# milos-agathon/forge3d

Hardware: AMD Instinct MI355X
Metric: Msamples/s (W*H*spp/s) at 1920x1080, 11616 spp (8 spp/frame x 1452 frames timed); SSIM vs golden (higher is better)
Workload: dtype f32

## Files before the change

forge3d_amd/_native.py:

```python
from __future__ import annotations

import ctypes as C
import os
from pathlib import Path

import numpy as np

_PKG = Path(__file__).resolve().parent
LIB_PATH = _PKG / "libf3dhip.so"

STATUS_OK, STATUS_VALUE, STATUS_RENDER, STATUS_UPLOAD, STATUS_DEVICE = 0, 1, 2, 3, 4
ABI_VERSION = 6
FRAMES_IN_FLIGHT_AUTO = 0xFFFFFFFF

_EARTH = {"flat": 0, "sphere": 1, "ellipsoid": 2, "wgs84": 2}
_REFRACTION = {"none": 0, "bennett": 1, "saemundsson": 2, "effective_radius": 3}


class Desc(C.Structure):
    _fields_ = [
        ("struct_size", C.c_uint32),
        ("heights", C.c_void_p), ("dem_width", C.c_uint32), ("dem_height", C.c_uint32),
        ("spacing_x", C.c_float), ("spacing_z", C.c_float), ("exaggeration", C.c_float),
        ("albedo", C.c_float * 3),
# ... 196 lines not shown
    ("f3d_scene_cache_entries", C.c_uint32, []),
    ("f3d_wavefront_render", C.c_int, [C.c_void_p, C.c_uint32, C.c_uint32, C.c_uint32, C.c_uint32, C.c_uint32, C.c_int32,
                                       C.c_void_p, C.c_char_p, C.c_size_t]),
    ("f3d_aether_bake", C.c_int, [C.c_void_p, C.c_void_p, C.c_void_p, C.c_void_p, C.c_void_p, C.c_void_p, _P(C.c_double),
                                  C.c_char_p, C.c_size_t]),
    ("f3d_smoke_render", C.c_int, [C.c_void_p, C.c_void_p, C.c_void_p, C.c_void_p, _P(C.c_double), C.c_char_p, C.c_size_t]),
    ("f3d_smoke_step", C.c_int, [C.c_void_p, C.c_void_p, C.c_void_p, C.c_uint32, C.c_uint32, _P(C.c_double), C.c_char_p, C.c_size_t]),
    ("f3d_aether_reference_render", C.c_int, [C.c_void_p, C.c_void_p, C.c_char_p, C.c_size_t]),
    ("f3d_smoke_composite", C.c_int, [C.c_void_p, C.c_void_p, _P(C.c_double), C.c_char_p, C.c_size_t]),
    ("f3d_session_fingerprint", C.c_int, [C.c_void_p, C.c_void_p, C.c_uint32]),
    ("f3d_session_mesh_tree", C.c_int, [C.c_void_p, _P(C.c_uint32), C.c_void_p, C.c_size_t, C.c_void_p, C.c_size_t, C.c_char_p, C.c_size_t]),
    ("f3d_session_rearm", C.c_int, [C.c_void_p, _P(RearmDesc), C.c_char_p, C.c_size_t]),
    ("f3d_session_render", C.c_int, [C.c_void_p, _P(Out), C.c_char_p, C.c_size_t]),
    ("f3d_session_reaim", C.c_int, [C.c_void_p, _P(ReaimDesc), C.c_char_p, C.c_size_t]),
    ("f3d_session_remesh", C.c_int, [C.c_void_p, _P(RemeshDesc), C.c_char_p, C.c_size_t]),
    ("f3d_session_reterrain", C.c_int, [C.c_void_p, _P(ReterrainDesc), C.c_char_p, C.c_size_t]),
    ("f3d_session_query", C.c_int, [C.c_void_p, _P(QueryDesc), C.c_char_p, C.c_size_t]),
    ("f3d_session_raster", C.c_int, [C.c_void_p, _P(RasterDesc), C.c_char_p, C.c_size_t]),
    ("f3d_session_horizon", C.c_int, [C.c_void_p, _P(HorizonDesc), C.c_char_p, C.c_size_t]),
    ("f3d_session_irradiation", C.c_int, [C.c_void_p, _P(IrradiationDesc), C.c_char_p, C.c_size_t]),
    ("f3d_session_drape", C.c_int, [C.c_void_p, _P(DrapeDesc), C.c_char_p, C.c_size_t]),
    ("f3d_session_draped", C.c_int, [C.c_void_p, _P(C.c_uint32)]),
    ("f3d_session_certificates", C.c_int, [C.c_void_p, _P(C.c_uint64)]),
    ("f3d_session_debug_wave_times", C.c_int, [C.c_void_p, C.c_void_p]),
    ("f3d_session_halo", C.c_int, [C.c_void_p, C.c_int32, C.c_int32, _P(C.c_void_p), _P(C.c_uint64)]),
    ("f3d_session_resolve", C.c_int, [C.c_void_p, C.c_uint32, C.c_void_p, C.c_void_p, C.c_void_p, C.c_void_p,
                                      _P(C.c_int32), C.c_char_p, C.c_size_t]),
    ("f3d_session_resolve_device", C.c_int, [C.c_void_p, C.c_uint32, C.c_void_p, C.c_void_p, C.c_void_p,
                                             C.c_void_p, C.c_char_p, C.c_size_t]),
    ("f3d_session_setup_ms", C.c_int, [C.c_void_p, _P(C.c_double), C.c_uint32]),
    ("f3d_session_info", C.c_int, [C.c_void_p, _P(C.c_uint64), _P(C.c_uint64), _P(C.c_uint64), _P(C.c_uint32),
                                   _P(C.c_uint32)]),
    ("f3d_session_kernel_timing", C.c_int, [C.c_void_p, C.c_int32, _P(C.c_double), _P(C.c_uint32)]),
    ("f3d_session_sample_lanes", C.c_uint32, [C.c_void_p]),
    ("f3d_session_row_costs", C.c_int, [C.c_void_p, _P(C.c_float), C.c_uint32, C.c_char_p, C.c_size_t]),
    ("f3d_session_primary_start", C.c_void_p, [C.c_void_p]),
    ("f3d_smoke_set_stream", None, [C.c_void_p]),
    ("f3d_smoke_wait_fields_read", C.c_int, [C.c_void_p]),
    ("f3d_smoke_seq_create", C.c_int, [C.c_void_p, C.c_void_p, _P(C.c_void_p), C.c_char_p, C.c_size_t]),
    ("f3d_smoke_seq_destroy", None, [C.c_void_p]),
    ("f3d_smoke_seq_streams", C.c_int, [C.c_void_p, _P(C.c_void_p), _P(C.c_void_p)]),
    ("f3d_smoke_seq_step", C.c_int, [C.c_void_p, C.c_void_p, C.c_void_p, C.c_void_p, C.c_uint32, C.c_uint32, _P(C.c_double), C.c_char_p, C.c_size_t]),
    ("f3d_smoke_seq_render", C.c_int, [C.c_void_p, C.c_void_p, C.c_void_p, C.c_void_p, C.c_void_p, _P(C.c_double), C.c_char_p, C.c_size_t]),
    ("f3d_smoke_seq_composite", C.c_int, [C.c_void_p, C.c_void_p, C.c_void_p, _P(C.c_double), C.c_char_p, C.c_size_t]),
    ("f3d_smoke_seq_stats", C.c_int, [C.c_void_p, C.c_void_p, C.c_char_p, C.c_size_t]),
    ("f3d_halo_rows", C.c_uint32, []),
# ... 325 lines not shown
```

forge3d_amd/csrc/f3d_frame.h:

```cpp
#pragma once
#include "f3d_launch.h"
#include "f3d_shade.h"
#include "f3d_query.h"
#include "f3d_raster.h"
#include "f3d_horizon.h"
#include "f3d_irradiation.h"
#include "f3d_lds.h"
#include "f3d_tiles.h"

namespace f3d {

template <uint32_t S = 1u>
__device__ __forceinline__ bool tile_pixel(const FrameParams &P, uint32_t &gx, uint32_t &gy, uint32_t &tile,
                                           const uint32_t *order = nullptr, uint32_t wg = 0xFFFFFFFFu) {
    if (wg == 0xFFFFFFFFu) wg = blockIdx.x;
    constexpr TileDims shape = tile_shape<S>();
    const uint32_t rows = P.band_end - P.band_begin;
    const TileGrid grid = tile_grid(P.cam.width, rows, shape);
    if (!workgroup_tile(wg, grid, P.tile_map, order, tile)) return false;
    tile_lane_pixel(tile, threadIdx.x, grid.tiles_x, P.band_begin, shape, gx, gy);
    return gx < P.cam.width && gy < P.band_end;
}
__device__ __forceinline__ bool tile_pixel(const FrameParams &P, uint32_t &gx, uint32_t &gy) {
    uint32_t tile;
    return tile_pixel<1u>(P, gx, gy, tile);
}
template <uint32_t S>
__device__ __forceinline__ void lane_pixel(const FrameParams &P, uint32_t tile, uint32_t &gx, uint32_t &gy) {
    constexpr TileDims shape = tile_shape<S>();
    tile_lane_pixel(tile, lane_now(), tiles_across(P.cam.width, shape), P.band_begin, shape, gx, gy);
}
// ... 458 lines not shown
    if (__ballot(redo) != 0ull) {
        LdsPending pend = make_pending(lds, P.terrain);
        if (redo) {
            m2 = fix_pixel(P, gx, gy, rec, pixels, pend);
            atomicAdd(&P.fix_count[2], 1u);
        }
    }
    if (P.collect_stats != 0u) publish_window_stats(P, active, m2);
}

__global__ __launch_bounds__(kWave) void k_trace_init(const FrameParams P) {
    uint32_t gx, gy;
    if (!tile_pixel(P, gx, gy)) return;
    const size_t lp = (size_t)(gy - P.row_begin) * P.cam.width + gx;
    P.head[lp] = first_head(P, P.gbuffer_n[lp]);
}

__device__ __forceinline__ bool head_neighbourhood_empty(const FrameParams &P, uint32_t gx, uint32_t gy) {
    const uint32_t lane = lane_now();
    const uint32_t x0 = gx - (lane & 7u), y0 = gy - (lane >> 3);
    const uint32_t x_last = (x0 + 7u < P.cam.width ? x0 + 7u : P.cam.width - 1u), y_last = (y0 + 7u < P.band_end ? y0 + 7u : P.band_end - 1u);
    const uint32_t xa = x0 >= kSpatialReachLo ? x0 - kSpatialReachLo : 0u, ya = y0 >= kSpatialReachLo ? y0 - kSpatialReachLo : 0u;
    static_assert(8u + kSpatialReachLo + kSpatialReachHi <= 16u, "the 16 x 16 raster below covers the tile's reach");
    const uint32_t xb = x_last + kSpatialReachHi < P.cam.width ? x_last + kSpatialReachHi : P.cam.width - 1u;
    const uint32_t yb = y_last + kSpatialReachHi < P.cam.height ? y_last + kSpatialReachHi : P.cam.height - 1u;
    const uint32_t *words = reinterpret_cast<const uint32_t *>(P.res_in);
    uint32_t some = 0u;
#pragma unroll
    for (uint32_t i = 0u; i < 4u; i++) {
        const uint32_t k = lane + 64u * i, bx = xa + (k & 15u), by = ya + (k >> 4);
        if (bx <= xb && by <= yb) some |= words[4u * reservoir_index(P, bx, by) + 1u] & ~kLightTypeBit;
    }
    return __ballot(some != 0u) == 0ull;
}

__global__ __launch_bounds__(kWave) void k_head(const FrameParams P) {
    uint32_t gx, gy, tile;
    const bool active = tile_pixel<1u>(P, gx, gy, tile);
    if (tile == 0xFFFFFFFFu) return;
#if !defined(F3D_NO_EMPTY_HEAD)
    if (P.frame_index > 0u && head_neighbourhood_empty(P, gx, gy)) {
        if (active) {
            const size_t ri = reservoir_index(P, gx, gy), lp = (size_t)(gy - P.row_begin) * P.cam.width + gx;
            const PackedReservoir self = P.res_in[ri];
            P.res_out[ri] = PackedReservoir{0.0f, self.m_lt, 0.0f, self.target_pdf};
            FrameHead h;
            h.centre_hit = P.gbuffer_n[lp].w != 0.0f;
            h.prev_valid = false;
            h.reuse_w = 1.0f;
            h.rng = 0u;
            P.head[lp] = pack_head(h);
        }
        return;
    }
#endif
    if (active) P.head[(size_t)(gy - P.row_begin) * P.cam.width + gx] = pack_head(frame_head<true>(P, gx, gy));
}

template <uint32_t S, bool MESH, bool DRAPE>
__device__ __forceinline__ void frame_wave(const FrameParams &P, uint32_t *lds) {
    const unsigned long long t_start = wall_clock64();
    typename PendingFor<MESH>::type pend{make_pending(lds, P.terrain)};
    uint32_t gx = 0u, gy = 0u, tile;
    const bool active = tile_pixel<S>(P, gx, gy, tile, P.tile_order);
    float m2 = 0.0f;
    if constexpr (S == 1u) {
        if (active) m2 = frame_pixel<DRAPE>(P, gx, gy, pend);
        if (P.collect_stats != 0u) publish_window_stats(P, active, m2);
    } else {
        m2 = frame_lanes<S, DRAPE>(P, tile, active, pend);
        if (P.collect_stats != 0u) publish_window_stats(P, active && (lane_now() & (S - 1u)) == 0u, m2);
    }
    if (lane_now() == 0u) {
        const unsigned long long t_end = wall_clock64();
        if (P.tile_cost && tile != 0xFFFFFFFFu) P.tile_cost[tile] = (uint32_t)(t_end - t_start);
#if defined(F3D_WAVE_TIMES)
        if (P.wave_times) {
            P.wave_times[2u * blockIdx.x] = t_start;
            P.wave_times[2u * blockIdx.x + 1u] = t_end;
        }
#endif
    }
}
template <int VARIANT, int MIN_WAVES = 1, uint32_t S = 1u, bool MESH = false>
__global__ __launch_bounds__(kWave, MIN_WAVES) void k_frame(const FrameParams P) {
    __shared__ __attribute__((aligned(16))) uint32_t lds[kLdsWords];
    frame_wave<S, MESH, false>(P, lds);
}
template <int MIN_WAVES, uint32_t S, bool MESH>
__global__ __launch_bounds__(kWave, MIN_WAVES) void k_frame_drape(const FrameParams P) {
    __shared__ __attribute__((aligned(16))) uint32_t lds[kLdsWords];
    frame_wave<S, MESH, true>(P, lds);
}

__global__ __launch_bounds__(kWave) void k_gbuffer(const FrameParams P, float4 *gbuffer_n, float *depth) {
    __shared__ __attribute__((aligned(16))) uint32_t lds[kLdsWords];
    LdsPending pend = make_pending(lds, P.terrain);
    uint32_t gx, gy;
    if (tile_pixel(P, gx, gy)) gbuffer_pixel(P, gx, gy, gbuffer_n, depth, pend);
}

__global__ __launch_bounds__(kWave) void k_rearm(const RearmParams R) {
    const FrameParams &P = R.frame;
    uint32_t gx, gy;
    if (!tile_pixel(P, gx, gy)) return;
    rearm_certificate(P, gx, gy, P.gbuffer_n, R.depth);
    rearm_clear(R, gx, gy);
    rearm_head(P, gx, gy, P.gbuffer_n[(size_t)(gy - P.row_begin) * P.cam.width + gx]);
}

__global__ __launch_bounds__(kWave) void k_reaim(const RearmParams R) {
    __shared__ __attribute__((aligned(16))) uint32_t lds[kLdsWords];
    LdsPending pend = make_pending(lds, R.frame.terrain);
    uint32_t gx, gy;
    if (tile_pixel(R.frame, gx, gy)) reaim_pixel(R, gx, gy, pend);
// ... 184 lines not shown
```

forge3d_amd/csrc/f3d_host.hip:

```cpp
#include <hip/hip_runtime.h>

#include <atomic>
#include <deque>
#include <exception>
#include <memory>
#include <map>
#include <mutex>
#include <new>
#include <unordered_map>

#include <unistd.h>

#include "f3d_bvh_refit.h"
#include "f3d_devmem.h"
#include "f3d_launch.h"
#include "f3d_lbvh.h"
#include "f3d_meshgrid.h"
#include "f3d_retable.h"
#include "f3d_setup.h"
#include "f3d_tables.h"
#include "f3d_tiles.h"

using namespace f3d;

namespace {

void hip_check(hipError_t e, const char *what) {
    if (e != hipSuccess) fail(F3D_STATUS_DEVICE, "HIP failure in %s: %s", what, hipGetErrorString(e));
}

struct DeviceGuard {
    int prev = -1;
    bool switched = false;
    explicit DeviceGuard(int device) {
        if (device < 0 || hipGetDevice(&prev) != hipSuccess) return;
        if (prev != device) switched = hipSetDevice(device) == hipSuccess;
    }
    ~DeviceGuard() {
        if (switched) (void)hipSetDevice(prev);
    }
};

template <class Body>
int c_abi(char *err, size_t errlen, Body &&body) {
// ... 92 lines not shown
    bool owns_reservoirs = false;
    uint8_t *d_rgba = nullptr;
    float *d_albedo = nullptr, *d_normal = nullptr;
    int variant = 0;
    AetherDev aether{};
    bool require_valid_reservoirs = false;
    f3d_terrain_ref_desc desc{};
    bool rendered = false;
    double reaim_seconds = 0.0;
    uint64_t budget = 0;
    struct Band {
        uint32_t begin = 0, end = 0;
        hipStream_t stream = nullptr;
        bool edge = true;
        hipEvent_t done[2] = {nullptr, nullptr};
        int64_t last = -1;
        bool unjoined = false;
    };
    std::vector<Band> bands;
    std::vector<hipStream_t> band_streams;
    hipEvent_t fork = nullptr;
    uint32_t *tile_cost = nullptr, *tile_order = nullptr;
    int64_t cost_frame = -1, order_frame = -1;
    uint32_t fd_frames = 0;
    bool wavefront = false;
    uint32_t wf_quorum = 0;
    int64_t trace_first = -1;
    uint32_t trace_count = 0;
    bool timing = false;
    std::vector<std::pair<hipEvent_t, hipEvent_t>> events;
    ~f3d_session() {
        for (auto &e : events) {
            (void)hipEventDestroy(e.first);
            (void)hipEventDestroy(e.second);
        }
        for (auto &b : bands)
            for (hipEvent_t e : b.done)
                if (e) (void)hipEventDestroy(e);
        if (fork) (void)hipEventDestroy(fork);
        for (hipStream_t st : band_streams) (void)hipStreamDestroy(st);
        if (host_stats) (void)hipHostFree(host_stats);
        for (auto &link : peer)
            for (void *base : link.opened)
                if (base) (void)hipIpcCloseMemHandle(base);
        if (halo_flags) (void)hipFree(halo_flags);
        mem.release();
    }
};

namespace {

void plan_bands(f3d_session &s, uint32_t want, uint32_t want_streams);

void aether_sun_terms(AetherDev &A, const f3d_terrain_ref_desc &d) {
    A.sun_intensity = aether_clamp_scale(f_clamp(d.sun_intensity, 0.0f, 65504.0f));
    A.exposure = aether_clamp_scale(f_clamp(d.exposure, 0.0f, 65504.0f));
}

uint32_t same_sun_of(const FrameParams &P) {
    return f_bits(P.light.wi.x) == f_bits(P.light.wi_reuse.x) && f_bits(P.light.wi.y) == f_bits(P.light.wi_reuse.y) &&
                   f_bits(P.light.wi.z) == f_bits(P.light.wi_reuse.z) ? 1u : 0u;
}

void upload_aether(f3d_session &s, const f3d_aether_luts &L, const f3d_terrain_ref_desc &d) {
    auto bad = [](const char *why) { fail(F3D_STATUS_RENDER, "invalid AETHER PT settings: %s", why); };
    const float scalars[9] = {L.turbidity, L.ozone_du, L.mie_g, L.bottom_radius_m, L.top_radius_m, L.rayleigh_scale_height_m,
                              L.mie_scale_height_m, L.max_aerial_distance_m, L.ground_albedo};
    for (float v : scalars)
        if (!std::isfinite(v)) bad("all scalar parameters must be finite");
    if (!(L.turbidity >= 1.0f && L.turbidity <= 10.0f)) bad("turbidity must be in [1, 10]");
    if (!(L.ozone_du >= 0.0f && L.ozone_du <= 600.0f)) bad("ozone must be in [0, 600] DU");
    if (!(L.mie_g >= 0.0f && L.mie_g <= 0.99f)) bad("mie_g must be in [0, 0.99]");
    if (L.bottom_radius_m <= 0.0f || L.top_radius_m <= L.bottom_radius_m) bad("top radius must exceed a positive bottom radius");
    if (L.rayleigh_scale_height_m <= 0.0f || L.mie_scale_height_m <= 0.0f || L.max_aerial_distance_m <= 0.0f)
        bad("scale heights and aerial distance must be positive");
    if (!(L.ground_albedo >= 0.0f && L.ground_albedo <= 1.0f)) bad("ground albedo must be in [0, 1]");
    if (L.scattering_orders < 2u || L.scattering_orders > 8u) bad("scattering_orders must be in [2, 8]");
    const uint32_t dims[9] = {L.transmittance_mu, L.transmittance_height, L.scattering_mu_view, L.scattering_mu_sun,
                              L.scattering_height, L.scattering_nu, L.aerial_distance, L.aerial_mu_view, L.aerial_height};
// ... 313 lines not shown

    if (s.mem.device_bytes > s.budget)
        fail(F3D_STATUS_RENDER,
             "terrain PT exceeds the memory budget before rendering: tracked total %llu (host-visible %llu) > limit %llu",
             (unsigned long long)s.mem.device_bytes, (unsigned long long)s.mem.host_visible_peak,
             (unsigned long long)s.budget);

    plan_bands(s, opts ? opts->bands : 0u, opts ? opts->band_streams : 0u);
    const bool lpt = s.bands.size() == 1 && ((s.variant / 1000) % 10 == 0);
    if ((s.variant / 1000) % 10 == 4) P.tile_map = 2u;
    if (lpt) {
        uint32_t grid = 0;
        const uint32_t tiles = frame_tile_count(P, &grid);
        s.tile_cost = (uint32_t *)s.mem.alloc((size_t)tiles * sizeof(uint32_t), "tile costs");
        s.tile_order = (uint32_t *)s.mem.alloc((size_t)(grid ? grid : 1u) * sizeof(uint32_t), "tile order");
        hip_check(hipMemsetAsync(s.tile_cost, 0, (size_t)tiles * sizeof(uint32_t), s.stream), "tile cost clear");
    }

    P.frame_index = 0;
    P.res_in = s.res[1];
    P.res_out = s.res[0];
    P.collect_stats = 0;
    hip_check(launch_gbuffer(P, s.gbuffer_n, s.depth, s.stream), "g-buffer pass");
    if (s.fd_frames) {
        P.band_begin = s.row_begin;
        P.band_end = s.row_end;
        hip_check(launch_trace_init(P, s.stream), "trace prediction init");
    }
    clock.lap(kSetupPasses);
}

template <class Launch>
void ordered_timed_launch(f3d_session &s, hipStream_t stream, uint32_t frame, Launch &&launch) {
    constexpr int64_t kOrderEvery = 4;
    FrameParams &P = s.params;
    P.tile_cost = s.tile_cost;
    P.tile_order = nullptr;
    if (s.tile_cost && s.cost_frame >= 0) {
        if (s.order_frame < 0 || s.cost_frame - s.order_frame >= kOrderEvery) {
            hip_check(launch_tile_order(P, s.tile_cost, s.tile_order, stream), "tile order kernel");
            s.order_frame = s.cost_frame;
        }
        P.tile_order = s.tile_order;
    }
    hipEvent_t e0 = nullptr, e1 = nullptr;
    if (s.timing) {
// ... 15 lines not shown
    FrameParams &P = s.params;
    P.frame_index = frame;
    P.res_out = s.res[frame & 1u];
    P.res_in = s.res[(frame & 1u) ^ 1u];
    P.collect_stats = collect ? 1u : 0u;
    P.band_begin = b.begin;
    P.band_end = b.end;
    const bool piped = b.stream != s.stream;
    if (b.last != (int64_t)frame - 1 && !(b.last < 0 && frame == 0u) && piped)
        fail(F3D_STATUS_VALUE, "frames must be enqueued in order (band %zu is at frame %lld, frame %u wanted)", index,
             (long long)b.last, frame);
    if (piped) {
        hip_check(hipStreamWaitEvent(b.stream, s.fork, 0), "band fork");
        for (int d = -1; d <= 1; d += 2) {
            const size_t n = index + (size_t)d;
            if (n >= s.bands.size() || frame == 0u) continue;
            f3d_session::Band &nb = s.bands[n];
            if (nb.last != (int64_t)frame - 1 && nb.last != (int64_t)frame)
                fail(F3D_STATUS_VALUE, "frames must be enqueued in order (band %zu is at frame %lld, frame %u wanted)", n,
                     (long long)nb.last, frame);
            if (nb.stream != b.stream) hip_check(hipStreamWaitEvent(b.stream, nb.done[(frame - 1u) & 1u], 0), "band wait");
        }
    }
    if (P.sample_lanes > 1u) hip_check(launch_head(P, b.stream), "frame head kernel");
    ordered_timed_launch(s, b.stream, frame, [&] { hip_check(launch_frame(P, s.variant, b.stream), "frame kernel"); });
    if (piped) {
        hip_check(hipEventRecord(b.done[frame & 1u], b.stream), "band done");
        b.unjoined = true;
    }
    b.last = frame;
    P.band_begin = s.row_begin;
    P.band_end = s.row_end;
}

void fork_bands(f3d_session &s, bool clear_stats) {
    if (clear_stats) hip_check(hipMemsetAsync(s.stats, 0, 2 * sizeof(uint32_t), s.stream), "stats clear");
    if (s.fork) hip_check(hipEventRecord(s.fork, s.stream), "band fork");
}

void join_bands(f3d_session &s, bool edges_only = false) {
    for (auto &b : s.bands)
        if (b.unjoined && (b.edge || !edges_only)) {
            hip_check(hipStreamWaitEvent(s.stream, b.done[b.last & 1], 0), "band join");
            b.unjoined = false;
        }
}

void refuse_draped(const f3d_session &s, const char *path) {
// ... 517 lines not shown
        const double t_setup = now_s();
        hip_check(hipStreamSynchronize(s->stream), "setup sync");
        out->setup_seconds = now_s() - t_setup + s->reaim_seconds;
        s->reaim_seconds = 0.0;
        render_loop(*s, out);
    });
}

int f3d_session_certificates(f3d_session *s, uint64_t out[2]) {
    if (!s || !out) return F3D_STATUS_VALUE;
    try {
        DeviceGuard guard(s->device);
        join_bands(*s);
        hip_check(hipStreamSynchronize(s->stream), "certificates");
        const size_t px = (size_t)s->rows * s->width;
        auto dev = [&](const void *ptr, size_t bytes) -> uint64_t {
            if (!ptr || !bytes) return 0ull;
            std::vector<uint8_t> host(bytes);
            hip_check(hipMemcpy(host.data(), ptr, bytes, hipMemcpyDeviceToHost), "certificate download");
            return hash_bytes(host.data(), bytes, 0x243F6A8885A308D3ull);
        };
        out[0] = dev(s->params.sun_clear, px * sizeof(float2));
        out[1] = dev(s->params.primary_start, px * sizeof(uint2));
        return F3D_STATUS_OK;
    } catch (...) {
        return F3D_STATUS_DEVICE;
    }
}

int f3d_session_debug_wave_times(f3d_session *s, void *device_buffer) {
#if defined(F3D_WAVE_TIMES)
    if (!s) return F3D_STATUS_VALUE;
    s->params.wave_times = (unsigned long long *)device_buffer;
    return F3D_STATUS_OK;
#else
    (void)s;
    (void)device_buffer;
    return F3D_STATUS_VALUE;
#endif
}

int f3d_terrain_ref_render(const f3d_terrain_ref_desc *desc, f3d_terrain_ref_out *out, char *err, size_t errlen) {
    if (err && errlen) err[0] = 0;
    if (!desc || !out) return F3D_STATUS_VALUE;
    f3d_session *s = new (std::nothrow) f3d_session();
    if (!s) return F3D_STATUS_DEVICE;
// ... 205 lines not shown
```

forge3d_amd/csrc/f3d_host_update.h:

```cpp
#pragma once

namespace {

struct Update {
    f3d_session &s;
    const bool cam;
    const double t_host = now_s();
    f3d_terrain_ref_desc d;
    FrameParams U{};
    bool require_valid = false;

    Update(f3d_session &session, const f3d_session_rearm_desc &r, const f3d_session_reaim_desc *aim, const char *done)
        : s(session), cam(aim != nullptr) {
        if (aim) check_struct_size(*aim, "f3d_session_reaim_desc");
        check_struct_size(r, "f3d_session_rearm_desc");
        if (s.peer[0].connected || s.peer[1].connected)
            fail(F3D_STATUS_VALUE, "a session with peer halos cannot be %s: the frame counters its neighbours poll only rise", done);
        d = s.desc;
        d.sun_azimuth_deg = r.sun_azimuth_deg;
        d.sun_elevation_deg = r.sun_elevation_deg;
        d.sun_intensity = r.sun_intensity;
        for (int c = 0; c < 3; c++) d.sun_color[c] = r.sun_color[c];
        d.exposure = r.exposure;
        d.env_intensity = r.env_intensity;
// ... 35 lines not shown
        s.require_valid_reservoirs = require_valid;
        s.desc = d;
        s.desc.mesh_vertices = nullptr;
        s.desc.mesh_indices = nullptr;

        join_bands(s);
        P.band_begin = s.row_begin;
        P.band_end = s.row_end;
        P.frame_index = 0;
        P.trace_first = 0u;
        P.res_in = s.res[1];
        P.res_out = s.res[0];
        P.collect_stats = 0;
        P.tile_order = nullptr;
        P.tile_cost = nullptr;
        RearmParams R{};
        R.frame = P;
        R.gbuffer_n = s.gbuffer_n;
        R.depth = s.depth;
        R.res[0] = s.res[0];
        R.res[1] = s.res[1];
        R.tile_cost = s.tile_cost;
        R.tiles = s.tile_cost ? frame_tile_count(P, nullptr) : 0u;
        if (cam) hip_check(launch_reaim(R, s.stream), "re-aim kernel");
        else hip_check(launch_rearm(R, s.stream), "re-arm kernel");
        s.cost_frame = s.order_frame = -1;
        s.rendered = false;
        s.trace_first = -1;
        s.trace_count = 0;
        for (auto &b : s.bands) {
            b.last = -1;
            b.unjoined = false;
        }
        s.reaim_seconds = cam ? now_s() - t_host : 0.0;
    }
};

void check_budget(const f3d_session &s, uint64_t planned, const char *update, const char *brings) {
    if (planned > s.budget)
        fail(F3D_STATUS_RENDER, "%s exceeds the memory budget: %s the tracked total to %llu > limit %llu", update, brings,
             (unsigned long long)planned, (unsigned long long)s.budget);
}

void rearm(f3d_session &s, const f3d_session_rearm_desc &r) {
    Update u(s, r, nullptr, "re-armed");
    u.validate();
    u.apply();
}
// ... 225 lines not shown
```

forge3d_amd/csrc/f3d_kernels.hip:

```cpp
#include <type_traits>

#include "f3d_frame.h"

namespace f3d {

void horizon_table_dims(uint32_t cell_w, uint32_t cell_h, uint32_t *level, uint32_t *bx, uint32_t *bz) {
    *level = horizon_block_level(cell_w, cell_h);
    *bx = (cell_w + (1u << *level) - 1u) >> *level;
    *bz = (cell_h + (1u << *level) - 1u) >> *level;
}
hipError_t launch_horizon_build(const TerrainDev &terrain, float *table, hipStream_t stream) {
    HorizonBuildParams B{};
    B.terrain = terrain;
    B.terrain.horizon = nullptr;
    horizon_table_dims(terrain.cell_w, terrain.cell_h, &B.level, &B.bx, &B.bz);
    B.table = table;
    hipLaunchKernelGGL(k_horizon_build, dim3(((B.bx + 7u) >> 3) * ((B.bz + 7u) >> 3)), dim3(kWave), 0, stream, B);
    return hipGetLastError();
}
static inline TileGrid band_tiles(const FrameParams &p, uint32_t lanes) {
    return tile_grid(p.cam.width, p.band_end - p.band_begin, tile_shape(lanes));
}
static inline uint32_t frame_grid(const FrameParams &p, uint32_t lanes = 1u) { return launch_size(band_tiles(p, lanes), p.tile_map); }

// ... 104 lines not shown
    hipLaunchKernelGGL(k_trace_init, dim3(frame_grid(p)), dim3(kWave), 0, stream, p);
    return hipGetLastError();
}
hipError_t launch_merge(const FrameParams &p, hipStream_t stream) {
    if (frame_grid(p) == 0u) return hipSuccess;
    hipLaunchKernelGGL(k_merge, dim3(frame_grid(p)), dim3(kWave), 0, stream, p);
    return hipGetLastError();
}
hipError_t launch_tile_order(const FrameParams &p, const uint32_t *cost, uint32_t *order, hipStream_t stream) {
    const TileGrid tiles = band_tiles(p, sample_lanes_of(p));
    TileOrderParams B{cost, order, tiles.tiles_x, tiles.tiles_y};
    hipLaunchKernelGGL(k_tile_order, dim3(kNumXcd), dim3(1024), 0, stream, B);
    return hipGetLastError();
}
uint32_t frame_tile_count(const FrameParams &p, uint32_t *grid) {
    const uint32_t lanes = sample_lanes_of(p);
    if (grid) *grid = frame_grid(p, lanes);
    return band_tiles(p, lanes).count();
}
hipError_t launch_gbuffer(const FrameParams &p, float4 *gbuffer_n, float *depth, hipStream_t stream) {
    hipLaunchKernelGGL(k_gbuffer, dim3(frame_grid(p)), dim3(kWave), 0, stream, p, gbuffer_n, depth);
    return hipGetLastError();
}
hipError_t launch_rearm(const RearmParams &p, hipStream_t stream) {
    if (frame_grid(p.frame) == 0u) return hipSuccess;
    hipLaunchKernelGGL(k_rearm, dim3(frame_grid(p.frame)), dim3(kWave), 0, stream, p);
    return hipGetLastError();
}
hipError_t launch_reaim(const RearmParams &p, hipStream_t stream) {
    if (frame_grid(p.frame) == 0u) return hipSuccess;
    hipLaunchKernelGGL(k_reaim, dim3(frame_grid(p.frame)), dim3(kWave), 0, stream, p);
    return hipGetLastError();
}
hipError_t launch_resolve(const ResolveParams &p, hipStream_t stream) {
    if (p.frame.drape) hipLaunchKernelGGL(k_resolve_drape, dim3(frame_grid(p.frame)), dim3(kWave), 0, stream, p);
    else hipLaunchKernelGGL(k_resolve, dim3(frame_grid(p.frame)), dim3(kWave), 0, stream, p);
    return hipGetLastError();
}
hipError_t launch_drape_pack(const DrapePackParams &p, hipStream_t stream) {
    if (p.rows == 0u || p.cols == 0u) return hipSuccess;
    hipLaunchKernelGGL(k_drape_pack, dim3((p.cols + 255u) / 256u, p.rows), dim3(256), 0, stream, p);
    return hipGetLastError();
}
hipError_t launch_ray_batch(const RayBatchParams &p, hipStream_t stream) {
    hipLaunchKernelGGL(k_ray_batch, dim3((p.n + kWave - 1) / kWave), dim3(kWave), 0, stream, p);
    return hipGetLastError();
// ... 56 lines not shown
```

forge3d_amd/csrc/f3d_launch.h:

```cpp
#pragma once

#include <hip/hip_runtime.h>

#include "f3d_aether.h"
#include "f3d_build.h"
#include "f3d_drape.h"
#include "f3d_scene.h"

namespace f3d {

struct RayBatchParams {
    TerrainDev terrain;
    const float4 *rays;
    uint32_t n;
    uint32_t any_hit, apply_curvature;
    uint32_t start_in_cell;
    uint32_t *out_hit;
    float *out_t;
    float *out_normal;
};

struct ResolveParams {
    FrameParams frame;
    uint32_t frames;
    uint8_t *rgba;
    float *albedo, *normal;
    AetherDev aether;
    const float *depth;
};

hipError_t launch_head(const FrameParams &p, hipStream_t stream);
hipError_t launch_frame(const FrameParams &p, int variant, hipStream_t stream);
hipError_t launch_trace(const FrameParams &p, uint32_t frames, hipStream_t stream);
hipError_t launch_trace_wavefront(const FrameParams &p, uint32_t frames, uint32_t quorum, hipStream_t stream);
hipError_t launch_merge(const FrameParams &p, hipStream_t stream);
hipError_t launch_trace_init(const FrameParams &p, hipStream_t stream);
uint32_t frame_tile_count(const FrameParams &p, uint32_t *grid);
hipError_t launch_tile_order(const FrameParams &p, const uint32_t *cost, uint32_t *order, hipStream_t stream);
hipError_t launch_gbuffer(const FrameParams &p, float4 *gbuffer_n, float *depth, hipStream_t stream);
hipError_t launch_rearm(const RearmParams &p, hipStream_t stream);
hipError_t launch_reaim(const RearmParams &p, hipStream_t stream);
hipError_t launch_resolve(const ResolveParams &p, hipStream_t stream);
hipError_t launch_drape_pack(const DrapePackParams &p, hipStream_t stream);
hipError_t launch_ray_batch(const RayBatchParams &p, hipStream_t stream);
hipError_t launch_query(const QueryParams &p, hipStream_t stream);
hipError_t launch_raster(const RasterParams &p, hipStream_t stream);
hipError_t launch_horizon(const HorizonParams &p, hipStream_t stream);
hipError_t launch_irradiation(const IrradiationParams &p, hipStream_t stream);
hipError_t launch_leaf_build(const PyramidBuildParams &p, hipStream_t stream);
hipError_t launch_level_build(const LevelBuildParams &p, hipStream_t stream);
hipError_t launch_band_build(const BandBuildParams &p, hipStream_t stream);
void horizon_table_dims(uint32_t cell_w, uint32_t cell_h, uint32_t *level, uint32_t *bx, uint32_t *bz);
hipError_t launch_horizon_build(const TerrainDev &terrain, float *table, hipStream_t stream);

}
```

forge3d_amd/csrc/f3d_scene.h:

```cpp
#pragma once

#include "f3d_math.h"

namespace f3d {

constexpr uint32_t kMaxLevels = 16;
constexpr uint32_t kRestirMCap = 512;
constexpr uint32_t kWelfordWindow = 32;
constexpr uint32_t kHaloRows = 4;
#if !defined(F3D_SPATIAL_REACH_HI)
#define F3D_SPATIAL_REACH_HI 4
#endif
constexpr uint32_t kSpatialReachLo = 3, kSpatialReachHi = F3D_SPATIAL_REACH_HI;
static_assert(kHaloRows >= kSpatialReachHi && kHaloRows >= kSpatialReachLo, "a strip's halo covers the spatial pass");
constexpr uint32_t kIblSectors = 8;
constexpr uint32_t kDefaultLeafQuorum = 64;

struct alignas(16) LeafRec {
    float h00, h10, h01, h11;
};
struct alignas(8) NodeRec {
    float mn, mx;
};

// ... 129 lines not shown
    const PackedReservoir *res_in;
    PackedReservoir *res_out;
    float4 *accum_mean;
    float *welford_m2;
    const float4 *gbuffer_n;
    uint32_t *stats;
    uint32_t collect_stats;
    uint32_t tile_map;
    uint32_t sample_lanes;
    uint2 *head;
    float2 *sun_clear;
    uint2 *primary_start;
    const uint32_t *tile_order;
    uint32_t *tile_cost;
    unsigned long long *wave_times;
    uint32_t band_begin, band_end;
    float4 *trace;
    uint32_t trace_first;
    uint32_t same_sun;
    uint32_t *fix_list;
    uint32_t *fix_count;
    WfQueues wf;
    const DrapeDev *drape;
};
F3D_HD uint32_t sample_lanes_of(const FrameParams &p) { return p.sample_lanes ? p.sample_lanes : 1u; }

struct RearmParams {
    FrameParams frame;
    float4 *gbuffer_n;
    float *depth;
    PackedReservoir *res[2];
    uint32_t *tile_cost;
    uint32_t tiles;
};

constexpr uint32_t kQueryClosest = 0u, kQueryOccluded = 1u, kQueryPixels = 2u;
struct QueryParams {
    FrameParams frame;
    uint32_t mode;
    uint32_t curved;
    uint32_t count;
    const float4 *rays;
    const uint2 *pixels;
    uint32_t *kind;
    float *t;
    float *normal;
// ... 46 lines not shown
```

forge3d_amd/csrc/f3d_shade.h:

```cpp
#pragma once

#include "f3d_aether.h"
#include "f3d_drape.h"
#include "f3d_march.h"
#include "f3d_trace.h"

namespace f3d {

struct SurfaceHit {
    float t;
    V3 p, n;
    uint32_t kind;
};


F3D_HD bool mesh_sweep(const MeshDev &M, V3 o, float tmin, V3 d, float tmax, float &t_best, V3 &n_best, uint32_t *tri_out = nullptr) {
    bool any = false;
    t_best = tmax;
    if (M.index_count < 3u) return false;
    for (uint32_t tri = 0u; tri + 2u < M.index_count; tri += 3u) {
        uint32_t i0 = M.indices[tri], i1 = M.indices[tri + 1u], i2 = M.indices[tri + 2u];
        if (i0 >= M.vertex_count || i1 >= M.vertex_count || i2 >= M.vertex_count) continue;
        float4 a = M.vertices[i0], b = M.vertices[i1], c = M.vertices[i2];
        float t;
// ... 685 lines not shown
    const IblRay q = sample_shade_sun<DRAPE>(P, h, ph, rng, o, pend);
    if (q.valid) o.b = q.b0 * (ibl_occluded(P, q.o, q.d, pend, q.t_stop) ? 0.0f : 1.0f);
    return o;
}

F3D_HD void accumulate_sample(Reservoir &cand, V3 &radiance, V3 a, V3 b, float target_pdf) {
    if (target_pdf > 0.0f) {
        cand.directional = true;
        cand.w_sum = cand.w_sum + target_pdf;
        cand.m = cand.m + 1u;
        cand.target_pdf = target_pdf;
    }
    radiance = (radiance + a) + b;
}

F3D_HD bool env_is_uniform(const EnvDev &E) { return E.width == 0u || E.height == 0u; }
F3D_HD V3 all_miss_radiance(const FrameParams &P) {
    const V3 a = env_radiance(P.env, V3{0.0f, 1.0f, 0.0f}), b = V3{0.0f, 0.0f, 0.0f};
    V3 radiance = V3{0.0f, 0.0f, 0.0f};
    for (uint32_t s = 0u; s < P.spp; s++) radiance = (radiance + a) + b;
    return radiance;
}

F3D_HD float frame_tail(const FrameParams &P, uint32_t gx, uint32_t gy, Reservoir cand, V3 radiance) {
    const size_t lp = (size_t)(gy - P.row_begin) * P.cam.width + gx;
    const float fspp = (float)P.spp;
    radiance = V3{radiance.x / fspp, radiance.y / fspp, radiance.z / fspp};
    if (cand.m > 0u && cand.w_sum > 0.0f && cand.target_pdf > 0.0f)
        cand.weight = restir_div(cand.w_sum, (float)cand.m * cand.target_pdf);
    const size_t ri = reservoir_index(P, gx, gy);
    const Reservoir prev = unpack(P.res_out[ri]);
    P.res_out[ri] = pack(temporal_merge(prev, cand));

    float4 am = P.accum_mean[lp];
    float wf_m2 = P.welford_m2[lp];
    float wf_mean = am.w;
    const V3 acc = V3{am.x + radiance.x, am.y + radiance.y, am.z + radiance.z};
    const float count = (float)(P.frame_index + 1u);
    const uint32_t phase = P.frame_index % kWelfordWindow;
    if (phase == 0u) {
        wf_mean = 0.0f;
        wf_m2 = 0.0f;
    }
    const float mean_lum = luminance(V3{acc.x / count, acc.y / count, acc.z / count});
    const float k = (float)phase + 1.0f;
    const float delta = mean_lum - wf_mean;
    const float mean = wf_mean + delta / k;
    const float m2 = f_fma(delta, mean_lum - mean, wf_m2);
    P.accum_mean[lp] = float4{acc.x, acc.y, acc.z, mean};
    P.welford_m2[lp] = m2;
    return m2;
}

F3D_HD float trace_code(bool hit, bool predicted_valid) { return (hit ? 1.0f : 0.0f) + (predicted_valid ? 2.0f : 0.0f); }
F3D_HD bool trace_code_hit(float code) { return code == 1.0f || code == 3.0f; }

template <class Pending>
F3D_HD void trace_pixel(const FrameParams &P, uint32_t frame, uint32_t gx, uint32_t gy, bool predicted_valid, float4 *rec,
                        size_t pixels, Pending &pend) {
    FrameHead h;
    h.centre_hit = false;
    h.prev_valid = predicted_valid;
    h.reuse_w = 1.0f;
    h.rng = P.cam.seed_hi ^ (gx * 1664525u) ^ (gy * 1013904223u) ^ (frame * 92837111u) ^ P.cam.seed_lo;
    uint32_t rng = h.rng;
    for (uint32_t s = 0u; s < P.spp; s++) {
        const PrimaryHit ph = sample_primary(P, gx, gy, rng, pend);
        rng = ph.rng;
        const SampleOut o = sample_shade(P, h, ph, rng, pend);
        rec[2u * (size_t)s * pixels] = float4{o.a.x, o.a.y, o.a.z, o.target_pdf};
        rec[2u * (size_t)s * pixels + 1u] = float4{o.b.x, o.b.y, o.b.z, trace_code(ph.hit.kind != 0u, predicted_valid)};
    }
}

// ... 217 lines not shown
```

forge3d_amd/session.py:

```python
from __future__ import annotations

import ctypes as C

import numpy as np

from . import _native

HALO_ROWS = 4
RESERVOIR_BYTES = 16
WELFORD_WINDOW = 32


class TerrainSession:
    def __init__(self, heightmap, width, height, camera=None, *, row_begin=0, row_end=0, device=-1, stream=0,
                 memory_budget_bytes=0, kernel_variant=0, ext_reservoirs=(None, None), ext_stats=None, bands=0,
                 band_streams=0, mesh_builder=0, frames_in_flight=0,
                 spacing=(1.0, 1.0), exaggeration=1.0, albedo=(0.6, 0.6, 0.6), sun_azimuth_deg=315.0,
                 sun_elevation_deg=45.0, sun_intensity=2.5, sun_color=(1.0, 0.97, 0.92), env_map=None,
                 env_intensity=0.35, mesh_vertices=None, mesh_indices=None, spp=1, max_frames=512, min_frames=32,
                 variance_threshold=1e-3, seed=7, observer_latitude_deg=0.0, observer_longitude_deg=0.0,
                 earth_model="ellipsoid", sphere_radius_m=6_371_008.8, refraction_model="bennett",
                 refraction_k=0.13, pressure_mbar=1013.25, temperature_c=15.0, atmosphere=None):
        self._lib = _native.lib()
        self._handle = C.c_void_p(None)
# ... 618 lines not shown
    def insolation(self, track, *, dni=None, dhi=None, azimuths=16, **irradiation_kwargs) -> dict:
        from . import insolation as _insolation

        unknown = set(irradiation_kwargs) - {"horizontal", "curved", "terrain_only", "lift", "region"}
        if unknown:
            raise TypeError(f"insolation() got unexpected keyword arguments {sorted(unknown)}")
        hours = np.asarray(track["hours"], np.float64)
        if dni is None or dhi is None:
            clear = _insolation.clear_sky(track["elevation_deg"])
            dni = clear[0] if dni is None else dni
            dhi = clear[1] if dhi is None else dhi
        dni, dhi = np.asarray(dni, np.float64), np.asarray(dhi, np.float64)
        direct = self.irradiation(np.asarray(track["directions"], np.float32), (dni * hours).astype(np.float32), **irradiation_kwargs)
        sky = {k: v for k, v in irradiation_kwargs.items() if k in ("curved", "lift", "region")}
        diffuse = (self.sky_view_factor(azimuths, **sky) * np.float32((dhi * hours).sum())).astype(np.float32)
        return {"direct": direct, "diffuse": diffuse, "global": (direct + diffuse).astype(np.float32)}

    def certificates(self) -> dict:
        out = (C.c_uint64 * 2)()
        if self._lib.f3d_session_certificates(self._handle, out) != 0:
            raise RuntimeError("f3d_session_certificates failed")
        return {"sun_clear": int(out[0]), "primary_start": int(out[1])}

    def enqueue_frames(self, first_frame: int, count: int, collect_stats: bool = False):
        self._check(self._lib.f3d_session_enqueue_frames(self._handle, int(first_frame), int(count),
                                                         1 if collect_stats else 0, self._err, len(self._err)))

    def enqueue_trace(self, first_frame: int, count: int):
        self._check(self._lib.f3d_session_enqueue_trace(self._handle, int(first_frame), int(count), self._err, len(self._err)))

    def enqueue_merge(self, frame: int, collect_stats: bool = False):
        self._check(self._lib.f3d_session_enqueue_merge(self._handle, int(frame), 1 if collect_stats else 0, self._err, len(self._err)))

    def frames_in_flight(self) -> int:
        return int(self._lib.f3d_session_frames_in_flight(self._handle))

    def trace_batch(self, frame: int, remaining: int) -> int:
        return int(self._lib.f3d_session_trace_batch(self._handle, int(frame), int(remaining)))

    def retraced_pixels(self) -> int:
        total = C.c_uint64(0)
        self._lib.f3d_session_retraced_pixels(self._handle, C.byref(total))
        return int(total.value)

    FINGERPRINT_FIELDS = ("camera", "light", "terrain_scalars", "mesh_scalars", "scalars", "leaf_table", "band_tables",
                          "mesh_vertices", "mesh_indices", "bvh_nodes", "bvh_triangles", "environment", "gbuffer",
# ... 173 lines not shown
```

include/f3d_terrain_pt.h:

```cpp
#ifndef F3D_TERRAIN_PT_H
#define F3D_TERRAIN_PT_H

#include <stddef.h>
#include <stdint.h>

#ifdef __cplusplus
extern "C" {
#endif

#define F3D_ABI_VERSION 6u
#define F3D_STATUS_OK 0
#define F3D_STATUS_VALUE 1
#define F3D_STATUS_RENDER 2
#define F3D_STATUS_UPLOAD 3
#define F3D_STATUS_DEVICE 4

#define F3D_EARTH_FLAT 0
#define F3D_EARTH_SPHERE 1
#define F3D_EARTH_ELLIPSOID 2
#define F3D_REFRACTION_NONE 0
#define F3D_REFRACTION_BENNETT 1
#define F3D_REFRACTION_SAEMUNDSSON 2
#define F3D_REFRACTION_EFFECTIVE_RADIUS 3

// ... 112 lines not shown
int f3d_session_halo_status(f3d_session *session, uint32_t *timeouts, char *err, size_t errlen);
int f3d_session_enqueue_batch_strip(f3d_session *session, uint32_t first_frame, uint32_t count, int32_t collect_stats_on_last,
                                    char *err, size_t errlen);
int f3d_session_resolve(f3d_session *session, uint32_t frames, uint8_t *rgba, float *albedo,
                        float *normal, float *depth, int32_t *any_valid_reservoir, char *err,
                        size_t errlen);
int f3d_session_set_accumulation(f3d_session *session, const float *sums_rgba, char *err, size_t errlen);
int f3d_session_resolve_device(f3d_session *session, uint32_t frames, void *d_rgba, void *d_albedo,
                               void *d_normal, void *d_depth, char *err, size_t errlen);
#define F3D_SETUP_PHASES 8
int f3d_session_setup_ms(f3d_session *session, double *out, uint32_t count);
typedef struct f3d_session_rearm_desc {
    uint32_t struct_size;
    float sun_azimuth_deg, sun_elevation_deg, sun_intensity;
    float sun_color[3];
    float exposure, env_intensity;
    uint32_t seed, max_frames, min_frames;
    float variance_threshold;
    double observer_latitude_deg, observer_longitude_deg, pressure_mbar, temperature_c;
} f3d_session_rearm_desc;
int f3d_session_rearm(f3d_session *session, const f3d_session_rearm_desc *desc, char *err, size_t errlen);
int f3d_session_render(f3d_session *session, f3d_terrain_ref_out *out, char *err, size_t errlen);
int f3d_session_certificates(f3d_session *session, uint64_t out[2]);
typedef struct f3d_session_reaim_desc {
    uint32_t struct_size;
    float cam_origin[3], cam_look_at[3], cam_up[3];
    float fov_y_deg;
    f3d_session_rearm_desc arm;
} f3d_session_reaim_desc;
int f3d_session_reaim(f3d_session *session, const f3d_session_reaim_desc *desc, char *err, size_t errlen);
typedef struct f3d_session_remesh_desc {
    uint32_t struct_size;
    const float *mesh_vertices;
    uint32_t mesh_vertex_count;
    const uint32_t *mesh_indices;
    uint32_t mesh_index_count;
    f3d_session_reaim_desc aim;
} f3d_session_remesh_desc;
int f3d_session_remesh(f3d_session *session, const f3d_session_remesh_desc *desc, char *err, size_t errlen);
typedef struct f3d_session_reterrain_desc {
    uint32_t struct_size;
    const float *heights;
    uint32_t width, height;
    uint32_t x0, y0;
    float exaggeration;
    f3d_session_reaim_desc aim;
// ... 278 lines not shown
```

Before: 9367.

## Skip frame work for deep-sky 8x8 blocks certified as sky

```diff
diff --git a/forge3d_amd/_native.py b/forge3d_amd/_native.py
--- a/forge3d_amd/_native.py
+++ b/forge3d_amd/_native.py
@@ -242,6 +242,7 @@
     ("f3d_session_drape", C.c_int, [C.c_void_p, _P(DrapeDesc), C.c_char_p, C.c_size_t]),
     ("f3d_session_draped", C.c_int, [C.c_void_p, _P(C.c_uint32)]),
     ("f3d_session_certificates", C.c_int, [C.c_void_p, _P(C.c_uint64)]),
+    ("f3d_session_sky_blocks", C.c_int, [C.c_void_p, _P(C.c_uint32)]),
     ("f3d_session_debug_wave_times", C.c_int, [C.c_void_p, C.c_void_p]),
     ("f3d_session_halo", C.c_int, [C.c_void_p, C.c_int32, C.c_int32, _P(C.c_void_p), _P(C.c_uint64)]),
     ("f3d_session_resolve", C.c_int, [C.c_void_p, C.c_uint32, C.c_void_p, C.c_void_p, C.c_void_p, C.c_void_p,
diff --git a/forge3d_amd/csrc/f3d_frame.h b/forge3d_amd/csrc/f3d_frame.h
--- a/forge3d_amd/csrc/f3d_frame.h
+++ b/forge3d_amd/csrc/f3d_frame.h
@@ -7,6 +7,7 @@
 #include "f3d_irradiation.h"
 #include "f3d_lds.h"
 #include "f3d_tiles.h"
+#include "f3d_skyblocks.h"
 
 namespace f3d {
 
@@ -511,6 +512,7 @@
     const uint32_t x_last = (x0 + 7u < P.cam.width ? x0 + 7u : P.cam.width - 1u), y_last = (y0 + 7u < P.band_end ? y0 + 7u : P.band_end - 1u);
     const uint32_t xa = x0 >= kSpatialReachLo ? x0 - kSpatialReachLo : 0u, ya = y0 >= kSpatialReachLo ? y0 - kSpatialReachLo : 0u;
     static_assert(8u + kSpatialReachLo + kSpatialReachHi <= 16u, "the 16 x 16 raster below covers the tile's reach");
+    static_assert(kSkyBlockMargin >= kSpatialReachLo && kSkyBlockMargin >= kSpatialReachHi, "a deep-sky block's margin covers the spatial pass");
     const uint32_t xb = x_last + kSpatialReachHi < P.cam.width ? x_last + kSpatialReachHi : P.cam.width - 1u;
     const uint32_t yb = y_last + kSpatialReachHi < P.cam.height ? y_last + kSpatialReachHi : P.cam.height - 1u;
     const uint32_t *words = reinterpret_cast<const uint32_t *>(P.res_in);
@@ -527,6 +529,12 @@
     uint32_t gx, gy, tile;
     const bool active = tile_pixel<1u>(P, gx, gy, tile);
     if (tile == 0xFFFFFFFFu) return;
+    if (P.sky_blocks != nullptr && (P.sky_blocks[tile] & kSkyBlockDeep) != 0u) {
+        float m2 = 0.0f;
+        if (active) m2 = frame_tail_accumulate(P, gx, gy, all_miss_radiance(P));
+        if (P.collect_stats != 0u) publish_window_stats(P, active, m2);
+        return;
+    }
 #if !defined(F3D_NO_EMPTY_HEAD)
     if (P.frame_index > 0u && head_neighbourhood_empty(P, gx, gy)) {
         if (active) {
@@ -549,9 +557,16 @@
 template <uint32_t S, bool MESH, bool DRAPE>
 __device__ __forceinline__ void frame_wave(const FrameParams &P, uint32_t *lds) {
     const unsigned long long t_start = wall_clock64();
-    typename PendingFor<MESH>::type pend{make_pending(lds, P.terrain)};
     uint32_t gx = 0u, gy = 0u, tile;
     const bool active = tile_pixel<S>(P, gx, gy, tile, P.tile_order);
+    if constexpr (S != 1u) {
+        if (P.sky_blocks != nullptr && tile != kNoTile) {
+            constexpr TileDims shape = tile_shape<S>();
+            const uint32_t block = sky_block_of_tile(tile, tiles_across(P.cam.width, shape), shape, tiles_across(P.cam.width, kSkyBlockShape));
+            if ((P.sky_blocks[block] & kSkyBlockDeep) != 0u) return;
+        }
+    }
+    typename PendingFor<MESH>::type pend{make_pending(lds, P.terrain)};
     float m2 = 0.0f;
     if constexpr (S == 1u) {
         if (active) m2 = frame_pixel<DRAPE>(P, gx, gy, pend);
@@ -580,6 +595,29 @@
 __global__ __launch_bounds__(kWave, MIN_WAVES) void k_frame_drape(const FrameParams P) {
     __shared__ __attribute__((aligned(16))) uint32_t lds[kLdsWords];
     frame_wave<S, MESH, true>(P, lds);
+}
+
+struct SkyBlocksParams {
+    const uint2 *primary_start;
+    uint32_t *blocks;
+    SkyBlockGeom geom;
+    uint32_t enabled;
+};
+__global__ __launch_bounds__(kWave) void k_sky_blocks(const SkyBlocksParams B) {
+    const uint32_t block = blockIdx.x;
+    const auto certified = [&](uint32_t x, uint32_t y) {
+        return certified_sky(B.primary_start[(size_t)(y - B.geom.row_begin) * B.geom.width + x]);
+    };
+    bool clear = false, own = false;
+    if (B.primary_start != nullptr) {
+        if (B.enabled != 0u) clear = sky_block_lane_clear(B.geom, block, threadIdx.x, certified);
+        const uint32_t x = (block % tiles_across(B.geom.width, kSkyBlockShape)) * 8u + (threadIdx.x & 7u);
+        const uint32_t y = B.geom.row_begin + (block / tiles_across(B.geom.width, kSkyBlockShape)) * 8u + (threadIdx.x >> 3);
+        own = x < B.geom.width && y < B.geom.row_end && certified(x, y);
+    }
+    const bool deep = __ballot(!clear) == 0ull;
+    const uint32_t count = (uint32_t)__popcll(__ballot(own));
+    if (threadIdx.x == 0u) B.blocks[block] = (deep ? kSkyBlockDeep : 0u) | (count << kSkyBlockCountShift);
 }
 
 __global__ __launch_bounds__(kWave) void k_gbuffer(const FrameParams P, float4 *gbuffer_n, float *depth) {
diff --git a/forge3d_amd/csrc/f3d_host.hip b/forge3d_amd/csrc/f3d_host.hip
--- a/forge3d_amd/csrc/f3d_host.hip
+++ b/forge3d_amd/csrc/f3d_host.hip
@@ -20,6 +20,7 @@
 #include "f3d_setup.h"
 #include "f3d_tables.h"
 #include "f3d_tiles.h"
+#include "f3d_skyblocks.h"
 
 using namespace f3d;
 
@@ -158,6 +159,7 @@
     hipEvent_t fork = nullptr;
     uint32_t *tile_cost = nullptr, *tile_order = nullptr;
     int64_t cost_frame = -1, order_frame = -1;
+    uint32_t *sky_blocks = nullptr;
     uint32_t fd_frames = 0;
     bool wavefront = false;
     uint32_t wf_quorum = 0;
@@ -191,6 +193,21 @@
 void aether_sun_terms(AetherDev &A, const f3d_terrain_ref_desc &d) {
     A.sun_intensity = aether_clamp_scale(f_clamp(d.sun_intensity, 0.0f, 65504.0f));
     A.exposure = aether_clamp_scale(f_clamp(d.exposure, 0.0f, 65504.0f));
+}
+
+bool sky_blocks_wanted(const f3d_session &s) {
+    return s.params.primary_start != nullptr && s.params.sample_lanes > 1u && s.fd_frames == 0u && s.bands.size() == 1;
+}
+bool sky_blocks_in_use(const f3d_session &s) {
+    const FrameParams &P = s.params;
+    return s.sky_blocks != nullptr && (P.env.width == 0u || P.env.height == 0u) && P.mesh.traversal_mode != 0u;
+}
+void enqueue_sky_blocks(f3d_session &s) {
+    if (!s.sky_blocks) return;
+    FrameParams P = s.params;
+    P.row_begin = s.row_begin;
+    P.row_end = s.row_end;
+    hip_check(launch_sky_blocks(P, s.sky_blocks, sky_blocks_in_use(s), s.stream), "sky-block table kernel");
 }
 
 uint32_t same_sun_of(const FrameParams &P) {
@@ -550,6 +567,10 @@
     P.res_out = s.res[0];
     P.collect_stats = 0;
     hip_check(launch_gbuffer(P, s.gbuffer_n, s.depth, s.stream), "g-buffer pass");
+    if (const size_t bytes = (size_t)std::max(sky_block_count(P), 1u) * sizeof(uint32_t); sky_blocks_wanted(s) && s.mem.device_bytes + bytes <= s.budget) {
+        s.sky_blocks = (uint32_t *)s.mem.alloc(bytes, "deep-sky blocks");
+        enqueue_sky_blocks(s);
+    }
     if (s.fd_frames) {
         P.band_begin = s.row_begin;
         P.band_end = s.row_end;
@@ -611,8 +632,10 @@
             if (nb.stream != b.stream) hip_check(hipStreamWaitEvent(b.stream, nb.done[(frame - 1u) & 1u], 0), "band wait");
         }
     }
+    P.sky_blocks = sky_blocks_in_use(s) && b.begin == s.row_begin && b.end == s.row_end ? s.sky_blocks : nullptr;
     if (P.sample_lanes > 1u) hip_check(launch_head(P, b.stream), "frame head kernel");
     ordered_timed_launch(s, b.stream, frame, [&] { hip_check(launch_frame(P, s.variant, b.stream), "frame kernel"); });
+    P.sky_blocks = nullptr;
     if (piped) {
         hip_check(hipEventRecord(b.done[frame & 1u], b.stream), "band done");
         b.unjoined = true;
@@ -1176,6 +1199,36 @@
         };
         out[0] = dev(s->params.sun_clear, px * sizeof(float2));
         out[1] = dev(s->params.primary_start, px * sizeof(uint2));
+        return F3D_STATUS_OK;
+    } catch (...) {
+        return F3D_STATUS_DEVICE;
+    }
+}
+
+int f3d_session_sky_blocks(f3d_session *s, uint32_t out[4]) {
+    if (!s || !out) return F3D_STATUS_VALUE;
+    try {
+        DeviceGuard guard(s->device);
+        join_bands(*s);
+        hip_check(hipStreamSynchronize(s->stream), "sky blocks");
+        FrameParams P = s->params;
+        P.row_begin = s->row_begin;
+        P.row_end = s->row_end;
+        const uint32_t blocks = sky_block_count(P), blocks_x = tiles_across(s->width, kSkyBlockShape);
+        out[0] = blocks;
+        out[1] = out[2] = out[3] = 0u;
+        if (!s->sky_blocks || blocks == 0u) return F3D_STATUS_OK;
+        std::vector<uint32_t> words(blocks);
+        hip_check(hipMemcpy(words.data(), s->sky_blocks, (size_t)blocks * sizeof(uint32_t), hipMemcpyDeviceToHost), "sky-block download");
+        const bool in_use = sky_blocks_in_use(*s);
+        for (uint32_t b = 0; b < blocks; b++) {
+            out[2] += words[b] >> kSkyBlockCountShift;
+            if (in_use && (words[b] & kSkyBlockDeep) != 0u) {
+                const uint32_t x0 = (b % blocks_x) * 8u, y0 = (b / blocks_x) * 8u;
+                out[1]++;
+                out[3] += std::min(8u, s->width - x0) * std::min(8u, s->rows - y0);
+            }
+        }
         return F3D_STATUS_OK;
     } catch (...) {
         return F3D_STATUS_DEVICE;
diff --git a/forge3d_amd/csrc/f3d_host_update.h b/forge3d_amd/csrc/f3d_host_update.h
--- a/forge3d_amd/csrc/f3d_host_update.h
+++ b/forge3d_amd/csrc/f3d_host_update.h
@@ -81,8 +81,12 @@
         R.res[1] = s.res[1];
         R.tile_cost = s.tile_cost;
         R.tiles = s.tile_cost ? frame_tile_count(P, nullptr) : 0u;
-        if (cam) hip_check(launch_reaim(R, s.stream), "re-aim kernel");
-        else hip_check(launch_rearm(R, s.stream), "re-arm kernel");
+        if (cam) {
+            hip_check(launch_reaim(R, s.stream), "re-aim kernel");
+            enqueue_sky_blocks(s);
+        } else {
+            hip_check(launch_rearm(R, s.stream), "re-arm kernel");
+        }
         s.cost_frame = s.order_frame = -1;
         s.rendered = false;
         s.trace_first = -1;
diff --git a/forge3d_amd/csrc/f3d_kernels.hip b/forge3d_amd/csrc/f3d_kernels.hip
--- a/forge3d_amd/csrc/f3d_kernels.hip
+++ b/forge3d_amd/csrc/f3d_kernels.hip
@@ -150,6 +150,15 @@
     hipLaunchKernelGGL(k_gbuffer, dim3(frame_grid(p)), dim3(kWave), 0, stream, p, gbuffer_n, depth);
     return hipGetLastError();
 }
+static inline SkyBlockGeom sky_geom(const FrameParams &p) { return SkyBlockGeom{p.cam.width, p.cam.height, p.row_begin, p.row_end}; }
+uint32_t sky_block_count(const FrameParams &p) { return sky_block_grid(sky_geom(p)).count(); }
+hipError_t launch_sky_blocks(const FrameParams &p, uint32_t *blocks, bool enabled, hipStream_t stream) {
+    const uint32_t count = sky_block_count(p);
+    if (count == 0u || !blocks) return hipSuccess;
+    const SkyBlocksParams B{p.primary_start, blocks, sky_geom(p), enabled ? 1u : 0u};
+    hipLaunchKernelGGL(k_sky_blocks, dim3(count), dim3(kWave), 0, stream, B);
+    return hipGetLastError();
+}
 hipError_t launch_rearm(const RearmParams &p, hipStream_t stream) {
     if (frame_grid(p.frame) == 0u) return hipSuccess;
     hipLaunchKernelGGL(k_rearm, dim3(frame_grid(p.frame)), dim3(kWave), 0, stream, p);
diff --git a/forge3d_amd/csrc/f3d_launch.h b/forge3d_amd/csrc/f3d_launch.h
--- a/forge3d_amd/csrc/f3d_launch.h
+++ b/forge3d_amd/csrc/f3d_launch.h
@@ -38,6 +38,8 @@
 uint32_t frame_tile_count(const FrameParams &p, uint32_t *grid);
 hipError_t launch_tile_order(const FrameParams &p, const uint32_t *cost, uint32_t *order, hipStream_t stream);
 hipError_t launch_gbuffer(const FrameParams &p, float4 *gbuffer_n, float *depth, hipStream_t stream);
+hipError_t launch_sky_blocks(const FrameParams &p, uint32_t *blocks, bool enabled, hipStream_t stream);
+uint32_t sky_block_count(const FrameParams &p);
 hipError_t launch_rearm(const RearmParams &p, hipStream_t stream);
 hipError_t launch_reaim(const RearmParams &p, hipStream_t stream);
 hipError_t launch_resolve(const ResolveParams &p, hipStream_t stream);
diff --git a/forge3d_amd/csrc/f3d_scene.h b/forge3d_amd/csrc/f3d_scene.h
--- a/forge3d_amd/csrc/f3d_scene.h
+++ b/forge3d_amd/csrc/f3d_scene.h
@@ -175,6 +175,7 @@
     uint32_t *fix_count;
     WfQueues wf;
     const DrapeDev *drape;
+    const uint32_t *sky_blocks;
 };
 F3D_HD uint32_t sample_lanes_of(const FrameParams &p) { return p.sample_lanes ? p.sample_lanes : 1u; }
 
diff --git a/forge3d_amd/csrc/f3d_shade.h b/forge3d_amd/csrc/f3d_shade.h
--- a/forge3d_amd/csrc/f3d_shade.h
+++ b/forge3d_amd/csrc/f3d_shade.h
@@ -731,16 +731,17 @@
     return radiance;
 }
 
-F3D_HD float frame_tail(const FrameParams &P, uint32_t gx, uint32_t gy, Reservoir cand, V3 radiance) {
-    const size_t lp = (size_t)(gy - P.row_begin) * P.cam.width + gx;
-    const float fspp = (float)P.spp;
-    radiance = V3{radiance.x / fspp, radiance.y / fspp, radiance.z / fspp};
+F3D_HD void frame_tail_reservoir(const FrameParams &P, uint32_t gx, uint32_t gy, Reservoir cand) {
     if (cand.m > 0u && cand.w_sum > 0.0f && cand.target_pdf > 0.0f)
         cand.weight = restir_div(cand.w_sum, (float)cand.m * cand.target_pdf);
     const size_t ri = reservoir_index(P, gx, gy);
     const Reservoir prev = unpack(P.res_out[ri]);
     P.res_out[ri] = pack(temporal_merge(prev, cand));
-
+}
+F3D_HD float frame_tail_accumulate(const FrameParams &P, uint32_t gx, uint32_t gy, V3 radiance) {
+    const size_t lp = (size_t)(gy - P.row_begin) * P.cam.width + gx;
+    const float fspp = (float)P.spp;
+    radiance = V3{radiance.x / fspp, radiance.y / fspp, radiance.z / fspp};
     float4 am = P.accum_mean[lp];
     float wf_m2 = P.welford_m2[lp];
     float wf_mean = am.w;
@@ -759,6 +760,10 @@
     P.accum_mean[lp] = float4{acc.x, acc.y, acc.z, mean};
     P.welford_m2[lp] = m2;
     return m2;
+}
+F3D_HD float frame_tail(const FrameParams &P, uint32_t gx, uint32_t gy, Reservoir cand, V3 radiance) {
+    frame_tail_reservoir(P, gx, gy, cand);
+    return frame_tail_accumulate(P, gx, gy, radiance);
 }
 
 F3D_HD float trace_code(bool hit, bool predicted_valid) { return (hit ? 1.0f : 0.0f) + (predicted_valid ? 2.0f : 0.0f); }
diff --git a/forge3d_amd/csrc/f3d_skyblocks.h b/forge3d_amd/csrc/f3d_skyblocks.h
--- /dev/null
+++ b/forge3d_amd/csrc/f3d_skyblocks.h
@@ -0,0 +1,49 @@
+#pragma once
+
+#include "f3d_tiles.h"
+
+namespace f3d {
+
+constexpr uint32_t kSkyBlockMargin = 4u;
+constexpr uint32_t kSkyBlockDeep = 1u, kSkyBlockCountShift = 8u;
+constexpr TileDims kSkyBlockShape = tile_shape<1u>();
+static_assert(kSkyBlockShape.log_w == 3u && kSkyBlockShape.log_h == 3u, "a block is 8 x 8 pixels");
+constexpr uint32_t kSkyBlockSpan = 8u + 2u * kSkyBlockMargin;
+static_assert(kSkyBlockSpan * kSkyBlockSpan == 4u * 64u, "a wave looks at the rectangle in four rounds of 64 lanes");
+
+struct SkyBlockGeom {
+    uint32_t width, height;
+    uint32_t row_begin, row_end;
+};
+F3D_HD constexpr TileGrid sky_block_grid(const SkyBlockGeom &g) { return tile_grid(g.width, g.row_end - g.row_begin, kSkyBlockShape); }
+
+constexpr uint32_t kSkySampleOutside = 0u, kSkySampleForeign = 1u, kSkySampleLookUp = 2u;
+F3D_HD uint32_t sky_block_sample(const SkyBlockGeom &g, uint32_t block, uint32_t k, uint32_t &x, uint32_t &y) {
+    const uint32_t blocks_x = tiles_across(g.width, kSkyBlockShape);
+    const int sx = (int)((block % blocks_x) * 8u) - (int)kSkyBlockMargin + (int)(k % kSkyBlockSpan);
+    const int sy = (int)(g.row_begin + (block / blocks_x) * 8u) - (int)kSkyBlockMargin + (int)(k / kSkyBlockSpan);
+    x = (uint32_t)sx;
+    y = (uint32_t)sy;
+    if (sx < 0 || sy < 0 || sx >= (int)g.width || sy >= (int)g.height) return kSkySampleOutside;
+    if (y < g.row_begin || y >= g.row_end) return kSkySampleForeign;
+    return kSkySampleLookUp;
+}
+
+template <class Certified>
+F3D_HD bool sky_block_lane_clear(const SkyBlockGeom &g, uint32_t block, uint32_t lane, Certified &&certified) {
+    bool clear = true;
+    for (uint32_t i = 0u; i < 4u; i++) {
+        uint32_t x, y;
+        const uint32_t where = sky_block_sample(g, block, lane + 64u * i, x, y);
+        if (where == kSkySampleForeign) clear = false;
+        else if (where == kSkySampleLookUp && !certified(x, y)) clear = false;
+    }
+    return clear;
+}
+
+F3D_HD uint32_t sky_block_of_tile(uint32_t tile, uint32_t tiles_x, TileDims d, uint32_t blocks_x) {
+    const uint32_t px = (tile % tiles_x) << d.log_w, py = (tile / tiles_x) << d.log_h;
+    return (py >> 3) * blocks_x + (px >> 3);
+}
+
+}
diff --git a/forge3d_amd/session.py b/forge3d_amd/session.py
--- a/forge3d_amd/session.py
+++ b/forge3d_amd/session.py
@@ -664,6 +664,12 @@
             raise RuntimeError("f3d_session_certificates failed")
         return {"sun_clear": int(out[0]), "primary_start": int(out[1])}
 
+    def sky_blocks(self) -> dict:
+        out = (C.c_uint32 * 4)()
+        if self._lib.f3d_session_sky_blocks(self._handle, out) != 0:
+            raise RuntimeError("f3d_session_sky_blocks failed")
+        return {"blocks": int(out[0]), "deep_blocks": int(out[1]), "certified_pixels": int(out[2]), "deep_pixels": int(out[3])}
+
     def enqueue_frames(self, first_frame: int, count: int, collect_stats: bool = False):
         self._check(self._lib.f3d_session_enqueue_frames(self._handle, int(first_frame), int(count),
                                                          1 if collect_stats else 0, self._err, len(self._err)))
diff --git a/include/f3d_terrain_pt.h b/include/f3d_terrain_pt.h
--- a/include/f3d_terrain_pt.h
+++ b/include/f3d_terrain_pt.h
@@ -158,6 +158,7 @@
 int f3d_session_rearm(f3d_session *session, const f3d_session_rearm_desc *desc, char *err, size_t errlen);
 int f3d_session_render(f3d_session *session, f3d_terrain_ref_out *out, char *err, size_t errlen);
 int f3d_session_certificates(f3d_session *session, uint64_t out[2]);
+int f3d_session_sky_blocks(f3d_session *session, uint32_t out[4]);
 typedef struct f3d_session_reaim_desc {
     uint32_t struct_size;
     float cam_origin[3], cam_look_at[3], cam_up[3];
```

New measurement: 9529, median of 6. 1.7% higher.
